# libv/cedarx_h264_encoder

Measured on NVIDIA B200. Metric: 1080p CQP I+P frames/sec (GOP-parallel), higher is better.
Workload: dtype u8

## Files before the change

cedarx_h264_encoder_b200/csrc/encoder.cu:

```cuda
#include "../../include/cedar_b200.h"
#include "cedar_headers.h"
#include "kernels.cuh"

#include <cuda_runtime.h>

#include <chrono>
#include <cstdio>
#include <cstdlib>
#include <cstring>
#include <errno.h>
#include <vector>

using namespace cedar;

#define ALIGN_UP(x, a) (((x) + ((a)-1)) & ~((size_t)(a)-1))

namespace {

enum KernelId {
    K_INGEST, K_ME, K_INTER, K_PINTRA, K_INTRA, K_BS, K_DEBLOCK, K_SSE, K_ESIZE, K_ESCAN, K_EZERO, K_EWRITE,
    K_CRESOLVE, K_CCODE, K_EPBCOUNT, K_EPBSCAN, K_PACKSCAN, K_EPBWRITE, K_COUNT
};
const char *kKernelNames[K_COUNT] = {
    "ingest_kernel", "me_kernel", "inter_kernel", "pintra_decide_kernel", "intra_kernel", "bs_kernel", "deblock_kernel",
// ... 288 lines not shown
        bins_per_mb = (24ull << 30) / ((size_t)g.nmb * F * sizeof(uint16_t));
        if (bins_per_mb < 160)
            bins_per_mb = 160;
    }
    if (const char *e = getenv("CEDAR_B200_BINS_PER_MB"))
        bins_per_mb = (size_t)atoll(e);
    bins_per_mb *= grow;
    h->eb.bins_cap = g.cabac ? (unsigned long long)(bins_per_mb * g.nmb + 8) * F + 64 : 0;
    h->eb.limb_cap = h->eb.rbsp_cap / 2 + 8;
    h->chunks_per_frame = (h->eb.rbsp_cap + EPB_CHUNK - 1) / EPB_CHUNK;
    if (clip)
        r |= hmalloc(&h->h_clip_out, h->out_cap);
    r |= dmalloc(&h->eb.rbsp, (size_t)h->eb.rbsp_cap * U);
    if (g.cabac) {
        r |= dmalloc(&h->eb.bins, (size_t)h->eb.bins_cap + 64);
        r |= dmalloc(&h->eb.limbs, (size_t)h->eb.limb_cap * L * S * (clip ? cedar_b200_handle::NSIDE : 1));
    }
    r |= dmalloc(&h->d_chunk_cnt, (size_t)h->chunks_per_frame * U);
    r |= dmalloc(&h->d_out, h->out_cap + 64);
    return r;
}

int alloc_buffers(cedar_b200_handle *h)
{
    const Geom &g = h->g;
    const int F = h->F, L = h->L;
    int r = 0;
    h->in_luma_size = (int)ALIGN_UP((size_t)g.src_w * g.src_h, 4096);
    size_t chroma_bytes = (size_t)g.src_w * g.src_h / (g.src_format == CEDAR_B200_FORMAT_NV16 ? 1 : 2);
    h->in_chroma_size = (int)ALIGN_UP(chroma_bytes, 4096);
    h->bytestream_size = (int)ALIGN_UP((size_t)g.nmb * 1536 + 4096, 4096);
    r |= hmalloc(&h->h_in_luma, h->in_luma_size);
    r |= hmalloc(&h->h_in_chroma, h->in_chroma_size);
    r |= hmalloc(&h->h_bytestream, h->bytestream_size);
    r |= hmalloc(&h->h_frame_bytes, F);
    r |= hmalloc(&h->h_total, 1);
    r |= hmalloc(&h->h_sse, F);
    r |= hmalloc(&h->h_error, 1);
    if (r)
        return r;

    const int S = h->S;
    const size_t U = (size_t)F * S;
    if (h->clip_mode)
        r |= hmalloc(&h->h_clip_in, h->raw_frame_bytes * F);
    r |= dmalloc(&h->d_raw, h->raw_frame_bytes * F + 64);
    r |= dmalloc(&h->d_src[0], g.frame_bytes * L);
    r |= dmalloc(&h->d_src[1], g.frame_bytes * L);
    r |= dmalloc(&h->d_unf, g.frame_bytes * L);
    r |= dmalloc(&h->d_rec[0], g.frame_bytes * L);
    r |= dmalloc(&h->d_rec[1], g.frame_bytes * L);
    for (int p = 0; p < 2; p++) {
        r |= dmalloc(&h->d_mbi[p], (size_t)g.nmb * L);
        r |= dmalloc(&h->d_nnz[p], (size_t)g.nmb * L * NNZ_STRIDE);
        r |= dmalloc(&h->d_i4[p], (size_t)g.nmb * L * 16);
        r |= dmalloc(&h->d_coef[p], (size_t)g.nmb * L * COEF_STRIDE);
    }
    r |= dmalloc(&h->d_flags, (size_t)3 * L * g.mbh);
    r |= dmalloc(&h->d_me_tabs, me_table_words(g.R, me_strip(g.R)));
    r |= dmalloc(&h->d_counters, 8 + 512);
    r |= dmalloc(&h->d_pwant, (size_t)g.nmb * L);
    r |= dmalloc(&h->d_pcount, (size_t)L);
    r |= dmalloc(&h->d_bs, (size_t)g.nmb * L * 32);
    r |= dmalloc(&h->d_sse, F);
    r |= dmalloc(&h->eb.mb_size, (size_t)L * (g.nmb + S + 1));
    r |= dmalloc(&h->eb.mb_off, (size_t)L * (g.nmb + S + 1));
    r |= dmalloc(&h->d_hdr_bits, (size_t)(F > h->K ? F : h->K) * S);
    r |= dmalloc(&h->d_hdr_nbits, (size_t)(F > h->K ? F : h->K) * S);
    r |= dmalloc(&h->eb.rbsp_len, U);
    r |= dmalloc(&h->eb.bins_cursor, 1);
    r |= dmalloc(&h->eb.bins_off, U);
    r |= dmalloc(&h->eb.bins_len, U);
    r |= dmalloc(&h->eb.error, 1);
    r |= dmalloc(&h->d_nal_bytes, U);
    r |= dmalloc(&h->d_nal_off, U);
    r |= dmalloc(&h->d_total, 1);
    r |= dmalloc(&h->d_frame_bytes, F);
    r |= alloc_entropy_buffers(h);
    if (r)
        return r;
    h->eb.hdr_bits = h->d_hdr_bits;
    h->eb.hdr_nbits = h->d_hdr_nbits;
    CK(cudaMemset(h->eb.error, 0, sizeof(int)));
    {
        std::vector<uint32_t> tabs(me_table_words(g.R, me_strip(g.R)));
        me_build_tables(g.R, me_strip(g.R), g.lambda, tabs.data());
        CK(cudaMemcpy(h->d_me_tabs, tabs.data(), tabs.size() * sizeof(uint32_t), cudaMemcpyHostToDevice));
    }
    CK(cudaMemset(h->d_counters, 0, sizeof(unsigned long long) * (8 + 512)));
    CK(cudaMemset(h->d_mbi[0], 0, sizeof(MbInfo) * g.nmb * L));
    CK(cudaMemset(h->d_mbi[1], 0, sizeof(MbInfo) * g.nmb * L));
    CK(cudaMemset(h->d_rec[0], 0, g.frame_bytes * L));
    CK(cudaMemset(h->d_rec[1], 0, g.frame_bytes * L));
    return 0;
}

void free_buffers(cedar_b200_handle *h)
{
    void *dev[] = {h->d_counters, h->d_raw, h->d_src[0], h->d_src[1], h->d_unf, h->d_rec[0], h->d_rec[1], h->d_mbi[0], h->d_mbi[1],
                   h->d_nnz[0], h->d_nnz[1], h->d_i4[0], h->d_i4[1], h->d_coef[0], h->d_coef[1], h->d_flags, h->d_me_tabs, h->d_pwant, h->d_pcount, h->d_bs,
                   h->d_sse, h->eb.mb_size, h->eb.mb_off, h->d_hdr_bits, h->d_hdr_nbits, h->eb.rbsp_len,
                   h->eb.bins_cursor, h->eb.bins_off, h->eb.bins_len, h->eb.error,
                   h->d_nal_bytes, h->d_nal_off, h->d_total, h->d_frame_bytes};
    free_entropy_buffers(h);
    for (void *p : dev)
        if (p)
            cudaFree(p);
    void *host[] = {h->h_in_luma, h->h_in_chroma, h->h_bytestream, h->h_frame_bytes, h->h_total, h->h_sse,
                    h->h_error, h->h_clip_in};
    for (void *p : host)
        if (p)
            cudaFreeHost(p);
}

static bool no_overlap_env()
{
    static const bool v = getenv("CEDAR_B200_NO_OVERLAP") != nullptr;
    return v;
}

int encode_step(cedar_b200_handle *h, const Step &s, int t, int gop_pos0, int step_index, bool wait_upload)
{
    const Geom &g = h->g;
    const int nl = s.nlanes, cur = t & 1, frame_i = t == 0, p = step_index & 1;
    const size_t flag_n = (size_t)h->L * g.mbh;
    int *fl_intra = h->d_flags, *fl_y = h->d_flags + flag_n, *fl_c = h->d_flags + 2 * flag_n;
    uint8_t *src = h->d_src[p], *unf = h->d_unf, *rec = h->d_rec[cur], *ref = h->d_rec[cur ^ 1];
    MbInfo *mbi = h->d_mbi[p];
    uint8_t *nnz = h->d_nnz[p], *bs = h->d_bs;
    int16_t *coef = h->d_coef[p];
    const bool no_overlap = no_overlap_env() || h->serialize;
    cudaStream_t st = h->stream, pre = no_overlap ? st : h->stream_pre, post = no_overlap ? st : h->stream_post;

    if (h->post_valid[p])
        CK(cudaStreamWaitEvent(pre, h->ev_post[p], 0));
    if (wait_upload)
        CK(cudaStreamWaitEvent(pre, h->ev_upload[h->upload_deferred_n ? step_index : t], 0));
    LAUNCH_ON(pre, K_INGEST, ingest_kernel, dim3((unsigned)((g.W / 16 + 127) / 128), (unsigned)(g.H + 2 * g.CH), nl), 128, 0, g, s, h->d_raw,
              h->raw_frame_bytes, src);
    CK(cudaEventRecord(h->ev_ingest[p], pre));

    CK(cudaStreamWaitEvent(st, h->ev_ingest[p], 0));
    if (h->post_valid[p])
        CK(cudaStreamWaitEvent(st, h->ev_post[p], 0));
    if (t == 0 && h->post_valid[p ^ 1])
        CK(cudaStreamWaitEvent(st, h->ev_post[p ^ 1], 0));
    CK(cudaMemsetAsync(h->d_flags, 0, sizeof(int) * 3 * flag_n, st));
    if (frame_i) {
        LAUNCH_ON(st, K_INTRA, intra_kernel, dim3((g.mbh + INTRA_ROWS - 1) / INTRA_ROWS, nl), INTRA_ROWS * 32, 0, g, s, src, unf,
                  mbi, nnz, coef, fl_intra, h->d_i4[p], nullptr, nullptr);
    } else {
        MeShape ms = me_shape(g.R);
        ms.noprune = h->no_prune;
        ms.exec_count = h->count ? h->d_counters : nullptr;
        const dim3 me_grid((g.mbw + ms.nstrip - 1) / ms.nstrip, (g.mbh + ms.nrow - 1) / ms.nrow, nl);
        const size_t me_smem = me_smem_bytes(g.R, ms.nstrip);
#define ME_LAUNCH(RSW_, COUNT_)                                                                                          \
    LAUNCH_ON(st, K_ME, (me_kernel<RSW_, COUNT_>), me_grid, ME_THREADS, me_smem, g, s, ms, src, ref, mbi, h->d_mbi[p ^ 1], h->d_me_tabs)
        if (h->count) {
            switch (ms.RSW) {
            case 27: ME_LAUNCH(27, true); break;
            case 43: ME_LAUNCH(43, true); break;
            default: ME_LAUNCH(0, true); break;
            }
        } else {
            switch (ms.RSW) {
            case 27: ME_LAUNCH(27, false); break;
            case 43: ME_LAUNCH(43, false); break;
            default: ME_LAUNCH(0, false); break;
            }
        }
#undef ME_LAUNCH
        LAUNCH_ON(st, K_INTER, inter_kernel, dim3((g.nmb + 3) / 4, nl), 128, 0, g, s, src, ref, unf, mbi, nnz, coef);
        if (g.p_intra) {
            CK(cudaMemsetAsync(h->d_pcount, 0, sizeof(int) * h->L, st));
            LAUNCH_ON(st, K_PINTRA, pintra_decide_kernel, dim3((g.nmb + 3) / 4, nl), 128, 0, g, s, src, unf, mbi, h->d_pwant,
                      h->d_pcount);
            LAUNCH_ON(st, K_INTRA, intra_kernel, dim3((g.mbh + INTRA_ROWS - 1) / INTRA_ROWS, nl), INTRA_ROWS * 32, 0, g, s, src, unf,
                      mbi, nnz, coef, fl_intra, h->d_i4[p], h->d_pwant, h->d_pcount);
        }
    }
    LAUNCH_ON(st, K_BS, bs_kernel, dim3((g.nmb * 8 + 127) / 128, nl), 128, 0, g, s, mbi, nnz, bs, !frame_i);
    CK(cudaEventRecord(h->ev_syn[p], st));
    const int db_ctas = (g.mbh + DB_ROWS - 1) / DB_ROWS, db_rows = (g.mbh + db_ctas - 1) / db_ctas;
    LAUNCH_ON(st, K_DEBLOCK, deblock_kernel, dim3((g.mbh + db_rows - 1) / db_rows, nl, 2), (db_rows + 2) * 32, 0, g, s, unf,
              rec, bs, fl_y, fl_c, db_rows);
    CK(cudaEventRecord(h->ev_main[p], st));

    CK(cudaStreamWaitEvent(post, h->ev_syn[p], 0));
    dim3 egrid((g.nmb + g.nslices + 127) / 128, nl);
    EntropyBufs eb = h->eb;
    eb.i4 = h->d_i4[p];
    LAUNCH_ON(post, K_ESIZE, entropy_size_kernel, egrid, 128, 0, g, s, frame_i, mbi, nnz, coef, eb);
    LAUNCH_ON(post, K_ESCAN, entropy_scan_kernel, dim3(1, nl), 1024, 0, g, s, h->eb);
    if (!g.cabac)
        LAUNCH_ON(post, K_EZERO, rbsp_zero_kernel, dim3(8, nl, g.nslices), 256, 0, s, h->eb.rbsp, h->eb.rbsp_cap,
                  h->eb.rbsp_len);
    LAUNCH_ON(post, K_EWRITE, entropy_write_kernel, egrid, 128, 0, g, s, frame_i, mbi, nnz, coef, eb);
    CK(cudaEventRecord(h->ev_ent[p], post));
    CK(cudaStreamWaitEvent(post, h->ev_main[p], 0));
    LAUNCH_ON(post, K_SSE, sse_kernel, dim3(32, nl), 256, 0, g, s, src, rec, h->d_sse);
    CK(cudaEventRecord(h->ev_post[p], post));
    h->post_valid[p] = true;
    if (g.cabac) {
        cudaStream_t side = no_overlap ? st : h->stream_cabac[h->side_next];
        CK(cudaStreamWaitEvent(side, h->ev_ent[p], 0));
        LAUNCH_ON(side, K_CRESOLVE, cabac_resolve_kernel, nl * g.nslices, RES_THREADS, RES_SMEM_BYTES, g, s, h->K, gop_pos0, h->eb,
                  h->count ? h->d_counters + 8 : nullptr);
        EntropyBufs ebc = h->eb;
        ebc.limbs += (size_t)(no_overlap || !h->clip_mode ? 0 : h->side_next) * h->L * g.nslices * h->eb.limb_cap;
        LAUNCH_ON(side, K_CCODE, cabac_code_kernel, nl * g.nslices, CP_THREADS, CP_SMEM_BYTES, g, s, ebc);
        if (!no_overlap) {
            h->side_used |= 1u << h->side_next;
            h->side_next = (h->side_next + 1) % cedar_b200_handle::NSIDE;
        }
    }
    h->last_cur = cur;
    h->last_par = p;
    return 0;
}

int finish_stream(cedar_b200_handle *h, int nframes, int gop_pos0, bool with_param_sets)
{
    CK(cudaEventRecord(h->ev_post_done, h->stream_post));
    CK(cudaStreamWaitEvent(h->stream, h->ev_post_done, 0));
    for (int i = 0; i < cedar_b200_handle::NSIDE; i++)
        if (h->side_used & (1u << i)) {
            CK(cudaEventRecord(h->ev_cabac[i], h->stream_cabac[i]));
            CK(cudaStreamWaitEvent(h->stream, h->ev_cabac[i], 0));
        }
    h->side_used = 0;
    unsigned cpf = h->chunks_per_frame;
    const int nunits = nframes * h->S;
    const unsigned cblocks = (cpf + 255) / 256;
    LAUNCH(K_EPBCOUNT, epb_count_kernel, (unsigned)nunits * cblocks, 256, 0, nunits, h->eb.rbsp, h->eb.rbsp_cap,
           h->eb.rbsp_len, h->d_chunk_cnt, cpf, cblocks);
    ParamSets ps;
    memset(&ps, 0, sizeof(ps));
    memcpy(ps.bytes, h->prefix, (size_t)h->prefix_len);
    ps.len = h->prefix_len;
    ps.mode = h->cfg.repeat_headers ? 2 : (with_param_sets ? 1 : 0);
    LAUNCH(K_EPBSCAN, epb_scan_kernel, nunits, 1024, 0, nunits, h->eb.rbsp_len, h->d_chunk_cnt, cpf, h->d_nal_bytes, ps, h->S,
           h->K, gop_pos0);
    LAUNCH(K_PACKSCAN, pack_scan_kernel, 1, 1024, 0, nunits, h->S, h->d_nal_bytes, 0u, h->d_nal_off, h->d_frame_bytes,
           h->d_total, (unsigned long long)h->out_cap, h->eb.error);
    LAUNCH(K_EPBWRITE, epb_write_kernel, (unsigned)nunits * cblocks, 256, 0, nunits, h->S, h->K, gop_pos0, h->eb.rbsp,
           h->eb.rbsp_cap, h->eb.rbsp_len, h->d_chunk_cnt, cpf, cblocks, h->d_nal_off, h->d_total, h->d_out, ps);
    return 0;
}

int build_header_table(cedar_b200_handle *h)
{
    const int S = h->S, rows = h->F > h->K ? h->F : h->K;
    std::vector<unsigned long long> bits((size_t)rows * S);
    std::vector<int> nbits((size_t)rows * S);
    for (int f = 0; f < rows; f++) {
        int p = f % h->K;
        for (int k = 0; k < S; k++) {
            uint64_t b = 0;
            int r = cedar_hdr_slice_mb(p == 0, p, h->g.cabac, k * h->g.srows * h->g.mbw, &b, &nbits[(size_t)f * S + k]);
            if (r)
                return r;
            bits[(size_t)f * S + k] = b;
        }
    }
    CK(cudaMemcpy(h->d_hdr_bits, bits.data(), sizeof(unsigned long long) * bits.size(), cudaMemcpyHostToDevice));
    CK(cudaMemcpy(h->d_hdr_nbits, nbits.data(), sizeof(int) * nbits.size(), cudaMemcpyHostToDevice));
    return 0;
}

int begin_stream(cedar_b200_handle *h, int nframes)
{
    CK(cudaMemsetAsync(h->eb.bins_cursor, 0, sizeof(unsigned long long), h->stream));
    CK(cudaMemsetAsync(h->d_sse, 0, sizeof(unsigned long long) * nframes, h->stream));
    CK(cudaMemsetAsync(h->eb.rbsp_len, 0, sizeof(uint32_t) * nframes * h->S, h->stream));
    CK(cudaMemsetAsync(h->eb.bins_len, 0, sizeof(uint32_t) * nframes * h->S, h->stream));
    CK(cudaEventRecord(h->ev_begin, h->stream));
    CK(cudaStreamWaitEvent(h->stream_pre, h->ev_begin, 0));
    CK(cudaStreamWaitEvent(h->stream_post, h->ev_begin, 0));
    h->post_valid[0] = h->post_valid[1] = false;
    return 0;
}

int check_error(cedar_b200_handle *h)
{
    if (*h->h_error) {
        fprintf(stderr, "cedar_b200: device buffer overflow (code %d): bitstream larger than the configured bound.\n",
                *h->h_error);
        cudaMemset(h->eb.error, 0, sizeof(int));
        return -ENOMEM;
    }
    return 0;
}

}

extern "C" {

const char *cedar_b200_version(void) { return "cedar_b200 0.1 (sm_100a)"; }

int cedar_b200_write_sps(const struct cedar_b200_config *cfg, uint8_t *out, int cap)
{
    const int wmb = (int)ALIGN_UP(cfg->dst_width, 16) >> 4, hmb = (int)ALIGN_UP(cfg->dst_height, 16) >> 4;
    return cedar_hdr_sps(cfg->profile, cfg->auto_level ? cedar_hdr_min_level(wmb * hmb) : cfg->level, wmb, hmb,
                         cfg->sps_crop ? (wmb * 16 - cfg->src_width) / 2 : 0,
                         cfg->sps_crop ? (hmb * 16 - cfg->src_height) / 2 : 0, out, cap);
// ... 602 lines not shown
```

cedarx_h264_encoder_b200/csrc/kernels.cuh:

```cuda
#pragma once
#include "entropy.cuh"
#include <cstdio>

namespace cedar {

struct Step {
    int nlanes;
    int frame0;
    int lane_stride;
    int nframes;
};
__device__ __forceinline__ int lane_frame(const Step &s, int lane)
{
    int f = s.frame0 + lane * s.lane_stride;
    return f < s.nframes ? f : -1;
}

__device__ __forceinline__ int ld_acquire(const int *p)
{
    int v;
    asm volatile("ld.acquire.gpu.global.s32 %0, [%1];" : "=r"(v) : "l"(p) : "memory");
    return v;
}
__device__ __forceinline__ void st_release(int *p, int v)
{
    asm volatile("st.release.gpu.global.s32 [%0], %1;" ::"l"(p), "r"(v) : "memory");
}

__device__ __forceinline__ uint32_t ingest_luma_word(const uint8_t *rp, int x, int src_w)
{
    if (x + 3 < src_w && !((uintptr_t)(rp + x) & 3))
        return *(const uint32_t *)(rp + x);
    uint32_t out = 0;
#pragma unroll
    for (int k = 0; k < 4; k++)
        out |= (uint32_t)rp[imin_(x + k, src_w - 1)] << (8 * k);
    return out;
}
__device__ __forceinline__ uint32_t ingest_chroma_word(const uint8_t *ra, const uint8_t *rb, int x, int c, int src_w, int nv16)
{
    uint32_t out = 0;
    if (2 * x + 7 < src_w && !(((uintptr_t)(ra + 2 * x) | (uintptr_t)(rb + 2 * x)) & 3)) {
        const uint32_t sel = c ? 0x7531u : 0x6420u;
        const uint32_t *pa = (const uint32_t *)(ra + 2 * x), *pb = (const uint32_t *)(rb + 2 * x);
        out = __byte_perm(pa[0], pa[1], sel);
        if (nv16)
            out = __vavgu4(out, __byte_perm(pb[0], pb[1], sel));
    } else {
#pragma unroll
        for (int k = 0; k < 4; k++) {
            const int sx = imin_(x + k, src_w / 2 - 1);
            const int a = ra[2 * sx + c], b = rb[2 * sx + c];
            out |= (uint32_t)((a + b + 1) >> 1) << (8 * k);
        }
    }
    return out;
}
__global__ void __launch_bounds__(128) ingest_kernel(Geom g, Step s, const uint8_t *__restrict__ raw, size_t raw_frame_bytes,
                                                     uint8_t *__restrict__ src)
{
    const int f = lane_frame(s, blockIdx.z);
    if (f < 0)
        return;
    const int row = blockIdx.y, x = (blockIdx.x * 128 + threadIdx.x) * 16;
    const uint8_t *luma = raw + (size_t)f * raw_frame_bytes;
    const uint8_t *chroma = luma + (size_t)g.src_w * g.src_h;
    uint8_t *dst = src + (size_t)blockIdx.z * g.frame_bytes;
    uint4 out;
    if (row < g.H) {
        if (x >= g.W)
            return;
        const uint8_t *rp = luma + (size_t)imin_(row, g.src_h - 1) * g.src_w;
        if (x + 15 < g.src_w && !((uintptr_t)(rp + x) & 15))
            out = *(const uint4 *)(rp + x);
        else
            out = make_uint4(ingest_luma_word(rp, x, g.src_w), ingest_luma_word(rp, x + 4, g.src_w),
                             ingest_luma_word(rp, x + 8, g.src_w), ingest_luma_word(rp, x + 12, g.src_w));
        *(uint4 *)(dst + (size_t)row * g.W + x) = out;
    } else {
        if (x >= g.CW)
            return;
        const int cr = row - g.H, c = cr >= g.CH, y = cr - (c ? g.CH : 0);
        const int sy = imin_(y, g.src_h / 2 - 1), nv16 = g.src_format == 1;
        const uint8_t *ra = chroma + (size_t)(nv16 ? 2 * sy : sy) * g.src_w, *rb = nv16 ? ra + g.src_w : ra;
        uint8_t *o = dst + (size_t)g.W * g.H + (size_t)c * g.CW * g.CH + (size_t)y * g.CW + x;
        if (x + 15 < g.CW && 2 * x + 31 < g.src_w && !(((uintptr_t)(ra + 2 * x) | (uintptr_t)(rb + 2 * x) | (uintptr_t)o) & 15)) {
            const uint32_t sel = c ? 0x7531u : 0x6420u;
            const uint4 a0 = ((const uint4 *)(ra + 2 * x))[0], a1 = ((const uint4 *)(ra + 2 * x))[1];
            out = make_uint4(__byte_perm(a0.x, a0.y, sel), __byte_perm(a0.z, a0.w, sel), __byte_perm(a1.x, a1.y, sel),
                             __byte_perm(a1.z, a1.w, sel));
            if (nv16) {
                const uint4 b0 = ((const uint4 *)(rb + 2 * x))[0], b1 = ((const uint4 *)(rb + 2 * x))[1];
                out.x = __vavgu4(out.x, __byte_perm(b0.x, b0.y, sel));
                out.y = __vavgu4(out.y, __byte_perm(b0.z, b0.w, sel));
                out.z = __vavgu4(out.z, __byte_perm(b1.x, b1.y, sel));
                out.w = __vavgu4(out.w, __byte_perm(b1.z, b1.w, sel));
            }
            *(uint4 *)o = out;
        } else {
#pragma unroll
            for (int k = 0; k < 4; k++)
                if (x + 4 * k < g.CW)
                    *(uint32_t *)(o + 4 * k) = ingest_chroma_word(ra, rb, x + 4 * k, c, g.src_w, nv16);
        }
    }
}

#define ME_THREADS 320
#define ME_MAX_STRIP 4
#define ME_MAX_ROWS 4
#define ME_MAX_MB (ME_MAX_STRIP * ME_MAX_ROWS)
#define ME_TASK_WORDS 1088

__device__ __forceinline__ uint32_t sad4_acc(uint32_t a, uint32_t b, uint32_t c)
{
    uint32_t d;
    asm("vabsdiff4.u32.u32.u32.add %0, %1, %2, %3;" : "=r"(d) : "r"(a), "r"(b), "r"(c));
    return d;
}

__host__ __device__ inline int me_strip(int R) { return R > 32 ? 2 : ME_MAX_STRIP; }
__host__ __device__ inline int me_rows(int R) { return R > 32 ? 1 : ME_MAX_ROWS; }
__host__ __device__ inline int me_row_words(int R, int nstrip)
{
    int w = (16 * nstrip + 2 * R + 3) / 4 + 2;
    return w | 1;
}
__host__ __device__ inline int me_window_rows(int R) { return 16 * me_rows(R) + 2 * R + (R < 2 ? 3 : 0); }
__host__ __device__ inline int me_copy_words(int R, int nstrip)
{
    int cw = me_window_rows(R) * me_row_words(R, nstrip);
    return cw + ((8 - (cw & 31)) & 31);
}
__host__ __device__ inline int me_item_words(int R, int nstrip)
{
    int nd = 2 * R + 1;
    return (((nd & 31) * ((nd + 3) >> 2) * nstrip * me_rows(R)) + 31) & ~31;
}
inline int me_group_row(int group, int nd)
{
    int oy0 = 4 * group;
    return oy0 + 4 <= nd ? oy0 : (nd >= 4 ? nd - 4 : 0);
}
inline size_t me_table_words(int R, int nstrip) { return 136 + ME_TASK_WORDS + me_item_words(R, nstrip); }
inline void me_build_tables(int R, int nstrip, int lambda, uint32_t *t)
{
    const int nd = 2 * R + 1, nfull = nd >> 5, nleft = nd & 31, ndyg = (nd + 3) >> 2, ntask_full = nfull * ndyg;
    for (int i = 0; i < 136; i++) {
        int d = i - R, a = d < 0 ? -d : d, bits = 1;
        if (a) {
            int lg = 0;
            while ((a >> lg) > 1)
                lg++;
            bits = 7 + 2 * lg;
        }
        t[i] = (uint32_t)(lambda * bits);
    }
    uint32_t *task = t + 136, *item = task + ME_TASK_WORDS;
    const int nmb = nstrip * me_rows(R);
    for (int i = 0; i < ntask_full * nmb; i++) {
        int m = i / ntask_full, k = i - m * ntask_full;
        task[i] = (uint32_t)m | ((uint32_t)((k / ndyg) * 32) << 4) | ((uint32_t)me_group_row(k % ndyg, nd) << 12);
    }
    const int per_mb = nleft * ndyg;
    for (int i = 0; i < me_item_words(R, nstrip); i++) {
        int m = per_mb ? i / per_mb : 0, jj = i - m * per_mb;
        item[i] = (per_mb && m < nmb) ? (uint32_t)m | ((uint32_t)(nfull * 32 + jj / ndyg) << 4) |
                                               ((uint32_t)me_group_row(jj % ndyg, nd) << 12)
                                         : 0xffffffffu;
    }
}
__host__ __device__ inline size_t me_smem_bytes(int R, int nstrip)
{
    return (size_t)(64 * nstrip * me_rows(R) + 4 * me_copy_words(R, nstrip) + me_item_words(R, nstrip)) * 4;
}

struct MeShape {
    int nstrip, lstrip, nrow, RSW, CWs, WR, nd, nfull, nleft, ndyg;
    int noprune;
    unsigned long long *exec_count;
};
inline MeShape me_shape(int R)
{
    MeShape m;
    m.nstrip = me_strip(R);
    m.lstrip = m.nstrip == 4 ? 2 : 1;
    m.nrow = me_rows(R);
    m.RSW = me_row_words(R, m.nstrip);
    m.CWs = me_copy_words(R, m.nstrip);
    m.WR = me_window_rows(R);
    m.nd = 2 * R + 1;
    m.nfull = m.nd >> 5, m.nleft = m.nd & 31, m.ndyg = (m.nd + 3) >> 2;
    m.noprune = 0;
    m.exec_count = nullptr;
    return m;
}

template <int kRSW, bool kCount = false>
__global__ void __launch_bounds__(ME_THREADS) me_kernel(Geom g, Step s, MeShape ms, const uint8_t *__restrict__ src,
                                                       const uint8_t *__restrict__ ref, MbInfo *__restrict__ mbi,
                                                       const MbInfo *__restrict__ mbi_prev,
                                                       const uint32_t *__restrict__ tabs)
{
    extern __shared__ uint32_t sm[];
    __shared__ uint32_t mb_best[ME_MAX_MB];
    __shared__ uint32_t mvcost[136];
    __shared__ uint32_t task_tab[ME_TASK_WORDS];
    if (lane_frame(s, blockIdx.z) < 0)
        return;
    const int R = g.R, nd = ms.nd, nstrip = ms.nstrip;
    const int WR = ms.WR, RSW = kRSW ? kRSW : ms.RSW, CWs = ms.CWs;
    const int mby0 = blockIdx.y * ms.nrow, mbx0 = blockIdx.x * nstrip, nmb = nstrip * ms.nrow, ls = ms.lstrip;
    const int ncols = imin_(nstrip, g.mbw - mbx0), nrows = imin_(ms.nrow, g.mbh - mby0);
    uint32_t vmask = 0;
#pragma unroll
    for (int m = 0; m < ME_MAX_MB; m++)
        vmask |= (uint32_t)(m < nmb && (m & (nstrip - 1)) < ncols && (m >> ls) < nrows) << m;
    const int x0 = mbx0 * 16, y0 = mby0 * 16;
    const uint8_t *srcY = src + (size_t)blockIdx.z * g.frame_bytes;
    const uint8_t *refY = ref + (size_t)blockIdx.z * g.frame_bytes;
    uint32_t *cur_s = sm, *cp = sm + 64 * nmb, *item_tab = cp + 4 * CWs;
    const int tid = threadIdx.x;

    const int nleft = ms.nleft, ndyg = ms.ndyg;
    const int ntask_full = ms.nfull * ndyg;
    const int nitems_left = nleft * ndyg * nmb;
    for (int i = tid; i < 136; i += ME_THREADS)
        mvcost[i] = tabs[i];
    for (int i = tid; i < ntask_full * nmb; i += ME_THREADS)
        task_tab[i] = tabs[136 + i];
    for (int i = tid; i < ((nitems_left + 31) & ~31); i += ME_THREADS)
        item_tab[i] = i < nitems_left ? tabs[136 + ME_TASK_WORDS + i] : 0xffffffffu;
    if (tid < ME_MAX_MB)
        mb_best[tid] = 0xffffffffu;
    for (int i = tid; i < 64 * nmb; i += ME_THREADS) {
        int m = i >> 6, row = (i >> 2) & 15, k = i & 3;
        if ((vmask >> m) & 1)
            cur_s[i] = *(const uint32_t *)(srcY + (size_t)(y0 + 16 * (m >> ls) + row) * g.W + x0 + 16 * (m & (nstrip - 1)) + 4 * k);
    }
    {
        const int warp_ = tid >> 5, lane_ = tid & 31;
        const bool interior_x = x0 - R >= 0 && x0 - R + 4 * RSW + 4 <= g.W && !((x0 - R) & 3);
        auto fetch = [&](const uint8_t *row, int k) -> uint32_t {
            const int fx = x0 - R + 4 * k;
            if (interior_x)
                return *(const uint32_t *)(row + fx);
            uint32_t v = 0;
#pragma unroll
            for (int i = 0; i < 4; i++)
                v |= (uint32_t)row[clip3_(0, g.W - 1, fx + i)] << (8 * i);
            return v;
        };
        const int nq = (RSW + 4) >> 2;
        const bool vec = interior_x && !((x0 - R) & 15) && RSW < 32 && x0 - R + 16 * nq <= g.W;
        if (vec) {
            const int sub = lane_ >> 3, q = lane_ & 7;
            for (int r4 = 4 * warp_; r4 < WR; r4 += 4 * (ME_THREADS / 32)) {
                const int r = r4 + sub;
                const bool on = r < WR && q < nq;
                uint4 v = make_uint4(0, 0, 0, 0);
                if (on)
                    v = *(const uint4 *)(refY + (size_t)clip3_(0, g.H - 1, y0 - R + r) * g.W + (x0 - R) + 16 * q);
                const uint32_t w[5] = {v.x, v.y, v.z, v.w, __shfl_down_sync(0xffffffffu, v.x, 1)};
                uint32_t *d = cp + r * RSW + 4 * q;
#pragma unroll
                for (int i = 0; i < 4; i++)
                    if (on && 4 * q + i < RSW) {
                        d[i] = w[i];
                        d[i + CWs] = __byte_perm(w[i], w[i + 1], 0x4321);
                        d[i + 2 * CWs] = __byte_perm(w[i], w[i + 1], 0x5432);
                        d[i + 3 * CWs] = __byte_perm(w[i], w[i + 1], 0x6543);
                    }
            }
        }
        for (int r = vec ? WR : warp_; r < WR; r += ME_THREADS / 32) {
            const uint8_t *row = refY + (size_t)clip3_(0, g.H - 1, y0 - R + r) * g.W;
            for (int k0 = 0; k0 < RSW; k0 += 32) {
                const int k = k0 + lane_;
                const uint32_t lo = k <= RSW ? fetch(row, k) : 0u;
                uint32_t hi = __shfl_down_sync(0xffffffffu, lo, 1);
                if (lane_ == 31 && k < RSW)
                    hi = fetch(row, k + 1);
                if (k < RSW) {
                    uint32_t *d = cp + r * RSW + k;
                    d[0] = lo;
                    d[CWs] = __byte_perm(lo, hi, 0x4321);
                    d[2 * CWs] = __byte_perm(lo, hi, 0x5432);
                    d[3 * CWs] = __byte_perm(lo, hi, 0x6543);
                }
            }
        }
    }
    __syncthreads();

    const int warp = tid >> 5, lane = tid & 31, nwarps = ME_THREADS / 32;
    for (int m = warp; m < nmb; m += nwarps) {
        const int mc = m & (nstrip - 1), mr = m >> ls, half = lane >> 4, l16 = lane & 15;
        if (!((vmask >> m) & 1))
            continue;
        int ox = R, oy = R;
        if (half) {
            const MbInfo pv = mbi_prev[(size_t)blockIdx.z * g.nmb + (size_t)(mby0 + mr) * g.mbw + mbx0 + mc];
            ox = clip3_(0, nd - 1, (pv.mv[0] >> 2) + R);
            oy = clip3_(0, nd - 1, (pv.mv[1] >> 2) + R);
        }
        uint32_t a = 0;
        const uint32_t *wp = cp + (ox & 3) * CWs + (oy + 16 * mr + l16) * RSW + 4 * mc + (ox >> 2);
        const uint32_t *cu = cur_s + 64 * m + 4 * l16;
#pragma unroll
        for (int k = 0; k < 4; k++)
            a = sad4_acc(wp[k], cu[k], a);
        a = __reduce_add_sync(half ? 0xffff0000u : 0x0000ffffu, a);
        if (l16 == 0)
            atomicMin(&mb_best[m], ((a + mvcost[ox] + mvcost[oy]) << 15) | (uint32_t)(oy * nd + ox));
    }
    __syncthreads();
    const int ntask = ntask_full * nmb + ((nitems_left + 31) >> 5);
    for (int task = warp; task < ntask; task += nwarps) {
        const uint32_t e = task < ntask_full * nmb ? task_tab[task] + ((uint32_t)lane << 4)
                                                   : item_tab[(task - ntask_full * nmb) * 32 + lane];
        uint32_t key = 0xffffffffu;
        const int m = (int)(e & 15);
        if (e != 0xffffffffu && ((vmask >> m) & 1)) {
            const int ox = (int)((e >> 4) & 255), oy0 = (int)(e >> 12);
            uint32_t cur[64];
            {
                const uint4 *c4 = (const uint4 *)(cur_s + 64 * m);
#pragma unroll
                for (int i = 0; i < 16; i++) {
                    uint4 v = c4[i];
                    cur[4 * i] = v.x, cur[4 * i + 1] = v.y, cur[4 * i + 2] = v.z, cur[4 * i + 3] = v.w;
                }
            }
            const uint32_t *wp = cp + (ox & 3) * CWs + (oy0 + 16 * (m >> ls)) * RSW + 4 * (m & (nstrip - 1)) + (ox >> 2);
            const uint32_t cx = mvcost[ox], rank0 = (uint32_t)(oy0 * nd + ox);
            uint32_t acc[4] = {cx + mvcost[oy0], cx + mvcost[oy0 + 1], cx + mvcost[oy0 + 2], cx + mvcost[oy0 + 3]};
            auto min_key = [&]() {
                uint32_t pm = 0xffffffffu;
#pragma unroll
                for (int j = 0; j < 4; j++) {
                    uint32_t k = acc[j] * 32768u + (rank0 + (uint32_t)(j * nd));
                    if (j == 3 && nd < 4)
                        k = 0xffffffffu;
                    pm = k < pm ? k : pm;
                }
                return pm;
            };
            bool dead = false;
            int rows_done = 19;
#pragma unroll
            for (int r = 0; r < 19; r++) {
                if ((r == 5 && kRSW == 43) || r == 9 || r == 13)
                    dead = min_key() > *(volatile uint32_t *)&mb_best[m] && !(kCount && ms.noprune);
                if (dead) {
                    if (kCount)
                        rows_done = r;
                    break;
                }
                uint32_t w0 = wp[r * RSW], w1 = wp[r * RSW + 1], w2 = wp[r * RSW + 2], w3 = wp[r * RSW + 3];
#pragma unroll
                for (int j = 0; j < 4; j++) {
                    int cr = r - j;
                    if (cr >= 0 && cr < 16) {
                        acc[j] = sad4_acc(w0, cur[cr * 4 + 0], acc[j]);
                        acc[j] = sad4_acc(w1, cur[cr * 4 + 1], acc[j]);
                        acc[j] = sad4_acc(w2, cur[cr * 4 + 2], acc[j]);
                        acc[j] = sad4_acc(w3, cur[cr * 4 + 3], acc[j]);
                    }
                }
            }
            if (!dead)
                key = min_key();
            if (kCount && ms.exec_count) {
                unsigned n4 = 0;
                for (int r = 0; r < rows_done; r++)
                    n4 += 4u * (unsigned)imin_(imin_(r + 1, 4), 19 - r);
                n4 = __reduce_add_sync(__activemask(), n4);
                if ((__activemask() & ((1u << lane) - 1)) == 0)
                    atomicAdd(ms.exec_count, (unsigned long long)n4);
            }
        }
        if (task < ntask_full * nmb) {
            key = __reduce_min_sync(0xffffffffu, key);
            if (lane == 0)
                atomicMin(&mb_best[m], key);
        } else if (key != 0xffffffffu)
            atomicMin(&mb_best[m], key);
    }
    __syncthreads();
    if (tid < nmb && ((vmask >> tid) & 1)) {
        const uint32_t b = mb_best[tid];
        int rank = (int)(b & 0x7fff);
        MbInfo mi;
        mi.type = MB_P16x16;
        mi.i16_mode = mi.chroma_mode = mi.cbp = 0;
        mi.mv[0] = (int16_t)((rank % nd - R) * 4);
        mi.mv[1] = (int16_t)((rank / nd - R) * 4);
        mi.mvd[0] = mi.mvd[1] = 0;
        mi.pad = b >> 15;
        mbi[(size_t)blockIdx.z * g.nmb + (size_t)(mby0 + (tid >> ls)) * g.mbw + mbx0 + (tid & (nstrip - 1))] = mi;
    }
}

struct ChromaOut {
    int zdc;
    int dcq;
    int cbpc;
    unsigned m_dc;
};

__device__ __forceinline__ ChromaOut chroma_dc_path(const int *w, int nz_ac, bool chroma, int lane, int qpc, int intra)
{
    ChromaOut o;
    const int base = 16 + ((lane - 16) & 4), cb = lane & 3;
    int d0 = __shfl_sync(0xffffffffu, w[0], base + 0), d1 = __shfl_sync(0xffffffffu, w[0], base + 1);
    int d2 = __shfl_sync(0xffffffffu, w[0], base + 2), d3 = __shfl_sync(0xffffffffu, w[0], base + 3);
    int qbits = 15 + qpc / 6, f = (1 << qbits) / (intra ? 3 : 6);
    o.zdc = chroma ? quant1(hadamard2x2_elem(cb, d0, d1, d2, d3), h264_quant_mf[qpc % 6][0], 2 * f, qbits + 1) : 0;
    unsigned m_ac = __ballot_sync(0xffffffffu, chroma && nz_ac > 0);
    o.m_dc = __ballot_sync(0xffffffffu, chroma && o.zdc != 0);
    o.cbpc = m_ac ? 2 : (o.m_dc ? 1 : 0);
    int z0 = __shfl_sync(0xffffffffu, o.zdc, base + 0), z1 = __shfl_sync(0xffffffffu, o.zdc, base + 1);
    int z2 = __shfl_sync(0xffffffffu, o.zdc, base + 2), z3 = __shfl_sync(0xffffffffu, o.zdc, base + 3);
    o.dcq = dequant_chroma_dc(hadamard2x2_elem(cb, z0, z1, z2, z3), qpc);
    return o;
}

__device__ __forceinline__ uint32_t pack4(const int *v)
{
    return (uint32_t)v[0] | ((uint32_t)v[1] << 8) | ((uint32_t)v[2] << 16) | ((uint32_t)v[3] << 24);
}

__device__ __forceinline__ void store_levels(int16_t *dst, const int16_t *lev)
{
    uint4 a, b;
    a.x = (uint16_t)lev[0] | ((uint32_t)(uint16_t)lev[1] << 16);
    a.y = (uint16_t)lev[2] | ((uint32_t)(uint16_t)lev[3] << 16);
    a.z = (uint16_t)lev[4] | ((uint32_t)(uint16_t)lev[5] << 16);
    a.w = (uint16_t)lev[6] | ((uint32_t)(uint16_t)lev[7] << 16);
    b.x = (uint16_t)lev[8] | ((uint32_t)(uint16_t)lev[9] << 16);
    b.y = (uint16_t)lev[10] | ((uint32_t)(uint16_t)lev[11] << 16);
    b.z = (uint16_t)lev[12] | ((uint32_t)(uint16_t)lev[13] << 16);
    b.w = (uint16_t)lev[14] | ((uint32_t)(uint16_t)lev[15] << 16);
    ((uint4 *)dst)[0] = a;
    ((uint4 *)dst)[1] = b;
}

struct LaneQuant {
    int mf[3], ls[3];
    int f, qbits, mul, rnd, sr;
};
__device__ __forceinline__ LaneQuant lane_quant_inter(int q)
{
    LaneQuant k;
    const int m = q % 6, e = q / 6;
#pragma unroll
    for (int c = 0; c < 3; c++) {
        k.mf[c] = h264_quant_mf[m][c];
        k.ls[c] = 16 * h264_dequant_v[m][c];
    }
    k.qbits = 15 + e;
    k.f = (1 << k.qbits) / 6;
    k.mul = e >= 4 ? 1 << (e - 4) : 1;
    k.rnd = e >= 4 ? 0 : 1 << (3 - e);
    k.sr = e >= 4 ? 0 : 4 - e;
    return k;
}

__global__ void __launch_bounds__(128) inter_kernel(Geom g, Step s, const uint8_t *__restrict__ src,
                                                    const uint8_t *__restrict__ ref, uint8_t *__restrict__ unf,
// ... 1972 lines not shown
```

Baseline: 14140.

## Add lower-bound pruning path to full-search motion estimation

Adds a bounded ME path that first builds a 4x4-downsampled table of the reference window and of the current MBs. It computes a SAD lower bound for every candidate and keeps only candidates that can beat the current best in a shared-memory list. Survivors get full SAD with an early-exit check halfway, and shifted window copies are built only if the list overflows, so exhaustive search is skipped in the common case. It also adds a minBlocks launch bound and uses funnel shifts instead of precomputed byte-shifted copies. The cost is extra table-building work, atomics on the list, and possible register pressure.

```diff
diff --git a/cedarx_h264_encoder_b200/csrc/encoder.cu b/cedarx_h264_encoder_b200/csrc/encoder.cu
--- a/cedarx_h264_encoder_b200/csrc/encoder.cu
+++ b/cedarx_h264_encoder_b200/csrc/encoder.cu
@@ -464,6 +464,8 @@
     } else {
         MeShape ms = me_shape(g.R);
         ms.noprune = h->no_prune;
+        if (h->count && h->no_prune)
+            ms.bound = 0;
         ms.exec_count = h->count ? h->d_counters : nullptr;
         const dim3 me_grid((g.mbw + ms.nstrip - 1) / ms.nstrip, (g.mbh + ms.nrow - 1) / ms.nrow, nl);
         const size_t me_smem = me_smem_bytes(g.R, ms.nstrip);
diff --git a/cedarx_h264_encoder_b200/csrc/kernels.cuh b/cedarx_h264_encoder_b200/csrc/kernels.cuh
--- a/cedarx_h264_encoder_b200/csrc/kernels.cuh
+++ b/cedarx_h264_encoder_b200/csrc/kernels.cuh
@@ -175,8 +175,23 @@
     return (size_t)(64 * nstrip * me_rows(R) + 4 * me_copy_words(R, nstrip) + me_item_words(R, nstrip)) * 4;
 }
 
+#define ME_LIST_CAP 2048
+__host__ __device__ inline int me_tab_pw(int R, int nstrip) { return ((16 * (nstrip - 1) + 2 * R + 12) >> 4) + 2; }
+__host__ __device__ inline int me_tab_rows(int R) { return me_window_rows(R) - 3; }
+__host__ __device__ inline int me_tab_words(int R, int nstrip) { return (me_tab_rows(R) + 3) * 4 * me_tab_pw(R, nstrip); }
+inline bool me_bound_path(int R)
+{
+    if (R < 2 || R > 32)
+        return false;
+    const int nstrip = me_strip(R);
+    return 4 * nstrip * me_rows(R) + me_tab_words(R, nstrip) + ME_LIST_CAP <= 3 * me_copy_words(R, nstrip);
+}
+
 struct MeShape {
     int nstrip, lstrip, nrow, RSW, CWs, WR, nd, nfull, nleft, ndyg;
+    int bound;
+    int tpw, trows;
+    uint32_t nd_magic;
     int noprune;
     unsigned long long *exec_count;
 };
@@ -191,13 +206,17 @@
     m.WR = me_window_rows(R);
     m.nd = 2 * R + 1;
     m.nfull = m.nd >> 5, m.nleft = m.nd & 31, m.ndyg = (m.nd + 3) >> 2;
+    m.bound = me_bound_path(R);
+    m.tpw = me_tab_pw(R, m.nstrip);
+    m.trows = me_tab_rows(R);
+    m.nd_magic = (uint32_t)(((1ull << 32) + (unsigned)m.nd - 1) / (unsigned)m.nd);
     m.noprune = 0;
     m.exec_count = nullptr;
     return m;
 }
 
 template <int kRSW, bool kCount = false>
-__global__ void __launch_bounds__(ME_THREADS) me_kernel(Geom g, Step s, MeShape ms, const uint8_t *__restrict__ src,
+__global__ void __launch_bounds__(ME_THREADS, kCount ? 1 : 4) me_kernel(Geom g, Step s, MeShape ms, const uint8_t *__restrict__ src,
                                                        const uint8_t *__restrict__ ref, MbInfo *__restrict__ mbi,
                                                        const MbInfo *__restrict__ mbi_prev,
                                                        const uint32_t *__restrict__ tabs)
@@ -206,6 +225,7 @@
     __shared__ uint32_t mb_best[ME_MAX_MB];
     __shared__ uint32_t mvcost[136];
     __shared__ uint32_t task_tab[ME_TASK_WORDS];
+    __shared__ int list_n;
     if (lane_frame(s, blockIdx.z) < 0)
         return;
     const int R = g.R, nd = ms.nd, nstrip = ms.nstrip;
@@ -238,7 +258,10 @@
         if ((vmask >> m) & 1)
             cur_s[i] = *(const uint32_t *)(srcY + (size_t)(y0 + 16 * (m >> ls) + row) * g.W + x0 + 16 * (m & (nstrip - 1)) + 4 * k);
     }
-    {
+    const bool bound = kRSW != 43 && ms.bound;
+    if (tid == 0)
+        list_n = 0;
+    auto stage = [&](const bool plain, const bool shifted) {
         const int warp_ = tid >> 5, lane_ = tid & 31;
         const bool interior_x = x0 - R >= 0 && x0 - R + 4 * RSW + 4 <= g.W && !((x0 - R) & 3);
         auto fetch = [&](const uint8_t *row, int k) -> uint32_t {
@@ -266,10 +289,13 @@
 #pragma unroll
                 for (int i = 0; i < 4; i++)
                     if (on && 4 * q + i < RSW) {
-                        d[i] = w[i];
-                        d[i + CWs] = __byte_perm(w[i], w[i + 1], 0x4321);
-                        d[i + 2 * CWs] = __byte_perm(w[i], w[i + 1], 0x5432);
-                        d[i + 3 * CWs] = __byte_perm(w[i], w[i + 1], 0x6543);
+                        if (plain)
+                            d[i] = w[i];
+                        if (shifted) {
+                            d[i + CWs] = __byte_perm(w[i], w[i + 1], 0x4321);
+                            d[i + 2 * CWs] = __byte_perm(w[i], w[i + 1], 0x5432);
+                            d[i + 3 * CWs] = __byte_perm(w[i], w[i + 1], 0x6543);
+                        }
                     }
             }
         }
@@ -283,15 +309,21 @@
                     hi = fetch(row, k + 1);
                 if (k < RSW) {
                     uint32_t *d = cp + r * RSW + k;
-                    d[0] = lo;
-                    d[CWs] = __byte_perm(lo, hi, 0x4321);
-                    d[2 * CWs] = __byte_perm(lo, hi, 0x5432);
-                    d[3 * CWs] = __byte_perm(lo, hi, 0x6543);
+                    if (plain)
+                        d[0] = lo;
+                    if (shifted) {
+                        d[CWs] = __byte_perm(lo, hi, 0x4321);
+                        d[2 * CWs] = __byte_perm(lo, hi, 0x5432);
+                        d[3 * CWs] = __byte_perm(lo, hi, 0x6543);
+                    }
                 }
             }
         }
-    }
+    };
+    stage(true, !bound);
     __syncthreads();
+    auto win = [&](const uint32_t *p, int sh) { return __funnelshift_r(p[0], p[1], sh); };
+    unsigned nabs = 0;
 
     const int warp = tid >> 5, lane = tid & 31, nwarps = ME_THREADS / 32;
     for (int m = warp; m < nmb; m += nwarps) {
@@ -305,17 +337,169 @@
             oy = clip3_(0, nd - 1, (pv.mv[1] >> 2) + R);
         }
         uint32_t a = 0;
-        const uint32_t *wp = cp + (ox & 3) * CWs + (oy + 16 * mr + l16) * RSW + 4 * mc + (ox >> 2);
+        const uint32_t *wp = cp + (oy + 16 * mr + l16) * RSW + 4 * mc + (ox >> 2);
         const uint32_t *cu = cur_s + 64 * m + 4 * l16;
 #pragma unroll
         for (int k = 0; k < 4; k++)
-            a = sad4_acc(wp[k], cu[k], a);
+            a = sad4_acc(win(wp + k, 8 * (ox & 3)), cu[k], a);
         a = __reduce_add_sync(half ? 0xffff0000u : 0x0000ffffu, a);
         if (l16 == 0)
             atomicMin(&mb_best[m], ((a + mvcost[ox] + mvcost[oy]) << 15) | (uint32_t)(oy * nd + ox));
     }
+    uint32_t *const qcur = cp + CWs, *const tab = qcur + 4 * nmb, *const list = tab + (ms.trows + 3) * 4 * ms.tpw;
+    const int tpw = ms.tpw, tw = 4 * tpw;
+    if (bound) {
+        if (tid < 4 * nmb && ((vmask >> (tid >> 2)) & 1)) {
+            const uint32_t *cu = cur_s + 16 * tid;
+            uint32_t q = 0;
+#pragma unroll
+            for (int j = 0; j < 4; j++) {
+                uint32_t a = 0;
+#pragma unroll
+                for (int r = 0; r < 4; r++)
+                    a = sad4_acc(cu[4 * r + j], 0u, a);
+                q |= (a >> 4) << (8 * j);
+            }
+            qcur[tid] = q;
+            if (kCount)
+                nabs += 16;
+        }
+        for (int i = tid; i < 3 * tw; i += ME_THREADS)
+            tab[ms.trows * tw + i] = 0;
+        constexpr int kSeg = 12;
+        const int xs_max = 16 * (nstrip - 1) + 2 * R + 12, nseg = (ms.trows + kSeg - 1) / kSeg;
+        for (int it = tid; it < nseg * tw; it += ME_THREADS) {
+            const int seg = it / tw, col = it - seg * tw, c = col / tpw, w = col - c * tpw;
+            const int y0 = seg * kSeg, y1 = imin_(y0 + kSeg, ms.trows), sh = 8 * c;
+            int idx[4];
+            uint32_t valid = 0;
+#pragma unroll
+            for (int j = 0; j < 4; j++) {
+                idx[j] = imin_(4 * w + j, RSW - 2);
+                valid |= (16 * w + c + 4 * j <= xs_max ? 0xffu : 0u) << (8 * j);
+            }
+            auto hrow = [&](int y, uint32_t *hh) {
+#pragma unroll
+                for (int j = 0; j < 4; j++)
+                    hh[j] = sad4_acc(win(cp + y * RSW + idx[j], sh), 0u, 0u);
+            };
+            auto put = [&](int y, const uint32_t *a, const uint32_t *b, const uint32_t *c_, const uint32_t *d) {
+                uint32_t q = 0;
+#pragma unroll
+                for (int j = 0; j < 4; j++)
+                    q |= ((a[j] + b[j] + c_[j] + d[j]) >> 4) << (8 * j);
+                tab[y * tw + col] = q & valid;
+            };
+            uint32_t h0[4], h1[4], h2[4], h3[4];
+            hrow(y0, h0), hrow(y0 + 1, h1), hrow(y0 + 2, h2);
+            for (int y = y0; y < y1; y += 4) {
+                hrow(y + 3, h3), put(y, h0, h1, h2, h3);
+                if (y + 1 < y1)
+                    hrow(y + 4, h0), put(y + 1, h1, h2, h3, h0);
+                if (y + 2 < y1)
+                    hrow(y + 5, h1), put(y + 2, h2, h3, h0, h1);
+                if (y + 3 < y1)
+                    hrow(y + 6, h2), put(y + 3, h3, h0, h1, h2);
+            }
+            if (kCount)
+                nabs += 4 * (y1 - y0 + 3);
+        }
+    }
     __syncthreads();
-    const int ntask = ntask_full * nmb + ((nitems_left + 31) >> 5);
+    bool fallback = !bound;
+    unsigned nbounded = 0, nsad = 0;
+    if (bound) {
+        const int nitem = nmb * 4 * nd;
+        for (int i0 = warp * 32; i0 < nitem; i0 += nwarps * 32) {
+            if (__shfl_sync(0xffffffffu, *(volatile int *)&list_n, 0) > ME_LIST_CAP)
+                break;
+            const int i = i0 + lane, t = (int)__umulhi((uint32_t)i, ms.nd_magic), ox = i - t * nd, c = t & 3;
+            const bool live = i < nitem && ((vmask >> (t >> 2)) & 1);
+            const int m = live ? t >> 2 : 0, x = 16 * (m & (nstrip - 1)) + ox, sh = 8 * ((x >> 2) & 3);
+            const uint32_t *tp = tab + (16 * (m >> ls) + c) * tw + (x & 3) * tpw + (x >> 4);
+            const uint4 q = ((const uint4 *)qcur)[m];
+            const uint32_t best = mb_best[m], cx = mvcost[ox] - 240u;
+            uint32_t w0 = win(tp, sh), w1 = win(tp + 4 * tw, sh), w2 = win(tp + 8 * tw, sh), pm = 0;
+            uint32_t rank = (uint32_t)(c * nd + ox);
+            for (int j = 0; j < ndyg; j++) {
+                const uint32_t w3 = win(tp + (4 * j + 12) * tw, sh);
+                uint32_t sb = sad4_acc(w0, q.x, 0u);
+                sb = sad4_acc(w1, q.y, sb);
+                sb = sad4_acc(w2, q.z, sb);
+                sb = sad4_acc(w3, q.w, sb);
+                const uint32_t key = (max(16u * sb, 240u) + cx + mvcost[c + 4 * j]) * 32768u + rank;
+                pm |= (uint32_t)(key <= best) << j;
+                rank += 4u * (uint32_t)nd;
+                w0 = w1, w1 = w2, w2 = w3;
+            }
+            pm &= live ? (1u << ((nd - c + 3) >> 2)) - 1u : 0u;
+            if (kCount && live)
+                nbounded += (nd - c + 3) >> 2;
+            while (__any_sync(0xffffffffu, pm)) {
+                const bool pass = pm != 0;
+                const int oy = c + 4 * (__ffs(pm) - 1);
+                pm &= pm - 1;
+                const uint32_t ball = __ballot_sync(0xffffffffu, pass);
+                int base = 0;
+                if (lane == 0)
+                    base = atomicAdd(&list_n, __popc(ball));
+                base = __shfl_sync(0xffffffffu, base, 0) + __popc(ball & ((1u << lane) - 1));
+                if (pass && base < ME_LIST_CAP)
+                    list[base] = (uint32_t)m | ((uint32_t)ox << 4) | ((uint32_t)oy << 12);
+            }
+        }
+        if (kCount)
+            nabs += 4 * nbounded;
+        __syncthreads();
+        fallback = list_n > ME_LIST_CAP;
+        if (!fallback) {
+            const int n = list_n;
+            for (int i = tid; i < n; i += ME_THREADS) {
+                const uint32_t e = list[i];
+                const int m = (int)(e & 15), ox = (int)((e >> 4) & 255), oy = (int)(e >> 12), sh = 8 * (ox & 3);
+                const uint32_t *wp = cp + (oy + 16 * (m >> ls)) * RSW + 4 * (m & (nstrip - 1)) + (ox >> 2);
+                const uint4 *cu = (const uint4 *)(cur_s + 64 * m);
+                const uint32_t rank = (uint32_t)(oy * nd + ox);
+                uint32_t acc = mvcost[ox] + mvcost[oy];
+                bool dead = false;
+#pragma unroll
+                for (int r = 0; r < 16; r++) {
+                    if (r == 8) {
+                        dead = ((acc << 15) | rank) > *(volatile uint32_t *)&mb_best[m];
+                        if (dead)
+                            break;
+                    }
+                    const uint4 cw = cu[r];
+                    const uint32_t *p = wp + r * RSW;
+                    acc = sad4_acc(win(p, sh), cw.x, acc);
+                    acc = sad4_acc(win(p + 1, sh), cw.y, acc);
+                    acc = sad4_acc(win(p + 2, sh), cw.z, acc);
+                    acc = sad4_acc(win(p + 3, sh), cw.w, acc);
+                }
+                if (kCount)
+                    nabs += dead ? 32 : 64, nsad++;
+                if (!dead)
+                    atomicMin(&mb_best[m], (acc << 15) | rank);
+            }
+        } else {
+            stage(false, true);
+            __syncthreads();
+        }
+    }
+    if (kCount && ms.exec_count && bound) {
+        const unsigned a = __reduce_add_sync(0xffffffffu, nabs), b = __reduce_add_sync(0xffffffffu, nbounded),
+                       c = __reduce_add_sync(0xffffffffu, nsad);
+        if (lane == 0) {
+            atomicAdd(ms.exec_count, (unsigned long long)a);
+            atomicAdd(ms.exec_count + 1, (unsigned long long)b);
+            atomicAdd(ms.exec_count + 2, (unsigned long long)c);
+        }
+        if (tid == 0) {
+            atomicAdd(ms.exec_count + 3, 1ull);
+            atomicAdd(ms.exec_count + 4, (unsigned long long)fallback);
+        }
+    }
+    const int ntask = fallback ? ntask_full * nmb + ((nitems_left + 31) >> 5) : 0;
     for (int task = warp; task < ntask; task += nwarps) {
         const uint32_t e = task < ntask_full * nmb ? task_tab[task] + ((uint32_t)lane << 4)
                                                    : item_tab[(task - ntask_full * nmb) * 32 + lane];
```

After: 15420 (median of 6 runs). 1.09x the previous value.
